# hellovuong/ORB_SLAM3_FAST

Measured on AMD Instinct MI355X. Metric: ORB extract+match frames/sec @1280×720 stereo (both-eye ORBextractor + ComputeStereoMatches), higher is better.
Workload: dtype u8; 1 GPU; C3: synthetic 1280x720 rectified stereo pairs, 1500 features, 8 levels, scale 1.2, FAST 20/7, ComputeStereoMatches (bf=0.12*532.03, b=0.12); handles=4, distinct_streams_per_gpu=32, frames_in_ring=3, stereo_matches_pair0=987, parallelism=independent stereo pairs sharded across GPUs, no data-path collective

## Files before the change

include/orbx.h:

```cpp
#ifndef ORBX_H_
#define ORBX_H_

#include <stddef.h>
#include <stdint.h>

#ifdef __cplusplus
extern "C" {
#endif

#define ORBX_MAX_LEVELS 12

#define ORBX_OK 0
#define ORBX_E_EMPTY (-1)
#define ORBX_E_BADARG (-2)
#define ORBX_E_CAPACITY (-3)
#define ORBX_E_HIP (-4)
#define ORBX_E_NODEVICE (-5)
#define ORBX_E_UNSUPPORTED (-6)
#define ORBX_E_TIMEOUT (-7)

typedef struct orbx_keypoint {
  float x, y, size, angle, response;
  int32_t octave, class_id;
} orbx_keypoint;
// ... 878 lines not shown
#define ORBX_GEOM_OPLUS 11
#define ORBX_GEOM_SIM3_EXP 12
#define ORBX_GEOM_SIM3_OPLUS 13
#define ORBX_GEOM_SO_INVERSE 14
#define ORBX_GEOM_RODRIGUES2ROT 15
#define ORBX_GEOM_ROT2RODRIGUES 16
#define ORBX_GEOM_OPS 17
#define ORBX_GEOM_MAX_ITEMS 65536
int orbx_debug_geometry(int device, int op, int n, const void* in, void* out);

void orbx_debug_set_detect_list_cap(int cap);
void orbx_debug_set_octree_global(int on);
void orbx_debug_set_octree_class(int nt);
int orbx_debug_octree_plan(const orbx_params* p, int width, int height, int32_t* nt_per_level, int32_t* lds_bytes_per_level);
void orbx_debug_set_stereo_direct(int max_pairs);
int orbx_debug_stereo_sort(orbx_extractor* left, int pair, int32_t* row_start, uint32_t* records, uint32_t* descriptors, int cap);
int orbx_debug_upload_results(orbx_extractor* ex, int image, const orbx_keypoint* kps, const uint8_t* desc, int n, int mono_index);
void orbx_debug_set_clahe_cell_kernel(int on);
void orbx_debug_set_remap_lds(int on);
int orbx_debug_remap_footprints(const float* map_x, const float* map_y, ptrdiff_t map_stride, int out_w, int out_h, int src_w,
                                int src_h, int n_maps, int32_t* table, int cap, int32_t* tiles_x, int32_t* tiles_y);
int orbx_debug_front_tables(const orbx_params* p, int width, int height, uint32_t* cells, int cells_cap, uint32_t* tiles,
                            int tiles_cap, int32_t info[4]);
int orbx_debug_preproc_plan(const orbx_preproc* pp, int32_t info[8]);
void orbx_debug_set_resize_tail(int first_level, int max_levels, int band_rows);
int orbx_debug_resize_plan(const orbx_extractor* ex, int32_t* first_level, int32_t* n_levels, int32_t* n_bands, int cap);
int orbx_debug_score_map(orbx_extractor* ex, int enable);
int orbx_debug_score_level(orbx_extractor* ex, int image, int level, uint8_t* dst, ptrdiff_t dst_stride);
int orbx_debug_sincos(int device, const float* angles, int n, int fused, float* sin_out, float* cos_out);
int orbx_debug_fast_atan2(int device, const float* y, const float* x, int n, float* out);
int orbx_debug_describe_plan(const orbx_params* p, int width, int height, int n_images, int32_t* out);
#define ORBX_SCRATCH_STATS 0
#define ORBX_SCRATCH_FILL 1
#define ORBX_SCRATCH_TRIM 2
int orbx_debug_scratch_pool(int device, int op, int byte, uint64_t* out);
int orbx_debug_fill_work_buffers(orbx_extractor* ex, int byte);

#ifdef __cplusplus
}
#endif
#endif
```

orb_slam3_fast_amd/__init__.py:

```python
import ctypes as C
import os

import numpy as np

_HERE = os.path.dirname(os.path.abspath(__file__))
LIB_PATH = os.path.join(_HERE, os.environ.get("ORBX_LIB_NAME", "liborbx.so"))

KP_DTYPE = np.dtype([("x", "<f4"), ("y", "<f4"), ("size", "<f4"), ("angle", "<f4"), ("response", "<f4"),
                     ("octave", "<i4"), ("class_id", "<i4")])
assert KP_DTYPE.itemsize == 28

OK, E_EMPTY, E_BADARG, E_CAPACITY, E_HIP, E_NODEVICE, E_UNSUPPORTED, E_TIMEOUT = 0, -1, -2, -3, -4, -5, -6, -7
TH_HIGH, TH_LOW, HISTO_LENGTH = 100, 50, 30
NUM_STAGES = 8
MP_DTYPE = np.dtype([("proj_x", "<f4"), ("proj_y", "<f4"), ("proj_xr", "<f4"), ("view_cos", "<f4"), ("track_depth", "<f4"),
                     ("predicted_level", "<i4"), ("in_view", "u1"), ("bad", "u1"), ("has_observations", "u1"),
                     ("pad_", "u1"), ("desc", "u1", (32,))])
assert MP_DTYPE.itemsize == 60
PP_DTYPE = np.dtype([("u", "<f4"), ("v", "<f4"), ("ur", "<f4"), ("radius", "<f4"), ("angle", "<f4"), ("min_level", "<i4"),
                     ("max_level", "<i4"), ("valid", "u1"), ("has_observations", "u1"), ("pad_", "u1", (2,)),
                     ("desc", "u1", (32,))])
assert PP_DTYPE.itemsize == 64
FP_DTYPE = np.dtype([("u", "<f4"), ("v", "<f4"), ("ur", "<f4"), ("radius", "<f4"), ("predicted_level", "<i4"), ("valid", "u1"),
                     ("pad_", "u1", (3,)), ("desc", "u1", (32,))])
# ... 186 lines not shown
                                                                       vp, vp]
        L.orbx_debug_inertial_linalg.argtypes = [i, i, i, vp, vp]
        L.orbx_debug_set_detect_list_cap.argtypes = [i]
        L.orbx_debug_set_detect_list_cap.restype = None
        L.orbx_debug_set_octree_global.argtypes = [i]
        L.orbx_debug_set_octree_global.restype = None
        if hasattr(L, "orbx_debug_set_octree_class"):
            L.orbx_debug_set_octree_class.argtypes = [i]
            L.orbx_debug_set_octree_class.restype = None
            L.orbx_debug_octree_plan.argtypes = [vp, i, i, vp, vp]
        L.orbx_debug_set_stereo_direct.argtypes = [i]
        L.orbx_debug_set_stereo_direct.restype = None
        if hasattr(L, "orbx_debug_stereo_sort"):
            L.orbx_debug_stereo_sort.argtypes = [vp, i, vp, vp, vp, i]
        L.orbx_debug_set_clahe_cell_kernel.argtypes = [i]
        L.orbx_debug_set_clahe_cell_kernel.restype = None
        L.orbx_debug_upload_results.argtypes = [vp, i, vp, vp, i, i]
        L.orbx_debug_set_remap_lds.argtypes = [i]
        L.orbx_debug_set_remap_lds.restype = None
        L.orbx_debug_remap_footprints.argtypes = [vp, vp, C.c_ssize_t, i, i, i, i, i, vp, i, C.POINTER(i), C.POINTER(i)]
        L.orbx_debug_preproc_plan.argtypes = [vp, vp]
        if hasattr(L, "orbx_debug_front_tables"):
            L.orbx_debug_front_tables.argtypes = [vp, i, i, vp, i, vp, i, vp]
        L.orbx_debug_set_resize_tail.argtypes = [i, i, i]
        L.orbx_debug_set_resize_tail.restype = None
        L.orbx_debug_resize_plan.argtypes = [vp, vp, vp, vp, i]
        L.orbx_debug_sincos.argtypes = [i, vp, i, i, vp, vp]
        if hasattr(L, "orbx_debug_fast_atan2"):
            L.orbx_debug_fast_atan2.argtypes = [i, vp, vp, i, vp]
            L.orbx_debug_describe_plan.argtypes = [vp, i, i, i, vp]
        L.orbx_debug_score_map.argtypes = [vp, i]
        L.orbx_set_opencv_compat.argtypes = [vp, i]
        L.orbx_debug_score_level.argtypes = [vp, i, i, vp, C.c_ssize_t]
        L.orbx_debug_scratch_pool.argtypes = [i, i, i, vp]
        L.orbx_debug_fill_work_buffers.argtypes = [vp, i]
        _lib = L
    return _lib


def _check(rc):
    if rc < 0:
        raise OrbxError(rc, lib().orbx_last_error().decode())
    return rc


def _p(a):
# ... 324 lines not shown
        _check(lib().orbx_debug_score_level(self._h, image, level, _p(out), w.value))
        return out

    def debug_resize_plan(self):
        a, b, c = (np.zeros(16, np.int32) for _ in range(3))
        n = _check(lib().orbx_debug_resize_plan(self._h, _p(a), _p(b), _p(c), 16))
        return [(int(a[i]), int(b[i]), int(c[i])) for i in range(n)]

    def debug_candidates(self, level, image=0):
        cap = 1 << 20
        out = np.zeros((cap, 3), np.int32)
        n = _check(lib().orbx_debug_candidates(self._h, image, level, _p(out), cap))
        return out[:n].copy()

    def debug_octree(self, width, height, candidates):
        counts, flat = _octree_candidates(candidates, self.nlevels)
        n = len(candidates)
        cap = int(self._nfeat.max()) + 64
        nsel = np.zeros(n * self.nlevels, np.int32)
        sel = np.zeros((n, self.nlevels, cap, 3), np.int32)
        _check(lib().orbx_debug_octree(self._h, int(width), int(height), n, _p(counts), _p(flat), _p(nsel), _p(sel), cap))
        return [[sel[i, l, :nsel[i * self.nlevels + l]].copy() for l in range(self.nlevels)] for i in range(n)]

    def debug_fill_work_buffers(self, byte):
        _check(lib().orbx_debug_fill_work_buffers(self._h, int(byte)))


SCRATCH_STATS, SCRATCH_FILL, SCRATCH_TRIM = 0, 1, 2


def scratch_pool_stats(device=0):
    out = np.zeros(4, np.uint64)
    _check(lib().orbx_debug_scratch_pool(int(device), SCRATCH_STATS, 0, _p(out)))
    return tuple(int(v) for v in out)


def scratch_pool_fill(byte, device=0):
    out = np.zeros(4, np.uint64)
    _check(lib().orbx_debug_scratch_pool(int(device), SCRATCH_FILL, int(byte), _p(out)))
    return int(out[0])


def scratch_pool_trim(device=0):
    _check(lib().orbx_debug_scratch_pool(int(device), SCRATCH_TRIM, 0, None))


# ... 1301 lines not shown
        raise ValueError("map_x and map_y must be float images of the same size")
    nm, dh, dw = mx.shape
    tx, ty = (dw + 127) // 128, (dh + 7) // 8
    tab = np.zeros((nm, tx, ty, 8), np.int32)
    gx, gy = C.c_int(), C.c_int()
    rc = lib().orbx_debug_remap_footprints(_p(mx), _p(my), dw, dw, dh, src_w, src_h, nm, _p(tab), tab.size, C.byref(gx), C.byref(gy))
    _check(rc)
    if (gx.value, gy.value) != (tx, ty):
        raise OrbxError("unexpected tile grid %d x %d" % (gx.value, gy.value))
    return tab if rc == 1 else None


def front_tables(nfeatures, scaleFactor, nlevels, iniThFAST, minThFAST, width, height):
    prm = _Params(int(nfeatures), float(scaleFactor), int(nlevels), int(iniThFAST), int(minThFAST))
    info = np.zeros(4, np.int32)
    _check(lib().orbx_debug_front_tables(C.byref(prm), width, height, None, 0, None, 0, _p(info)))
    cells = np.zeros((int(info[0]), 16), np.uint32)
    tiles = np.zeros(int(info[1]), np.uint32)
    _check(lib().orbx_debug_front_tables(C.byref(prm), width, height, _p(cells), cells.size, _p(tiles) if tiles.size else None,
                                         tiles.size, _p(info)))
    return cells, tiles, int(info[2]), int(info[3])


def octree_plan(nfeatures, scaleFactor, nlevels, iniThFAST, minThFAST, width, height):
    prm = _Params(int(nfeatures), float(scaleFactor), int(nlevels), int(iniThFAST), int(minThFAST))
    nt, lds = np.zeros(int(nlevels), np.int32), np.zeros(int(nlevels), np.int32)
    _check(lib().orbx_debug_octree_plan(C.byref(prm), width, height, _p(nt), _p(lds)))
    return nt, lds


def _octree_candidates(candidates, nlevels):
    counts, parts = [], [np.zeros((0, 3), np.int32)]
    for per_level in candidates:
        if len(per_level) != nlevels:
            raise ValueError("one candidate array per level")
        for c in per_level:
            c = np.asarray(c, np.int32).reshape(-1, 3)
            counts.append(len(c))
            parts.append(c)
    return np.array(counts, np.int32), np.ascontiguousarray(np.concatenate(parts))


def octree_check(nfeatures, scaleFactor, nlevels, iniThFAST, minThFAST, width, height, candidates):
    prm = _Params(int(nfeatures), float(scaleFactor), int(nlevels), int(iniThFAST), int(minThFAST))
    counts, flat = _octree_candidates(candidates, int(nlevels))
    _check(lib().orbx_debug_octree_check(C.byref(prm), int(width), int(height), len(candidates), _p(counts), _p(flat)))
# ... 521 lines not shown
```

orb_slam3_fast_amd/csrc/orbx_api.hip:

```cpp
#include "orbx_host.h"
#include "orbx_rgbd.h"

namespace orbx_host {
thread_local std::string g_err;
}

namespace {
struct StageTimer {
  orbx_extractor* ex;
  hipStream_t s;
  int stage;
  size_t i0 = 0;
  bool on;
  StageTimer(orbx_extractor* ex_, hipStream_t s_, int stage_)
      : ex(ex_), s(s_), stage(stage_), on(ex_->profiling && (ex_->profStage < 0 || ex_->profStage == stage_)) {
    if (!on) {
      if (s == ex->stream) ex->lastEvValid = false;
      return;
    }
    if (s == ex->stream && ex->lastEvValid) {
      i0 = ex->lastEv;
    } else {
      hipEvent_t e = ex->next_event();
      i0 = ex->evCursor - 1;
// ... 167 lines not shown
        const int ce = std::min((int)xtab[D.xcoef + x1].x + 1, S.w - 1);
        const int ndw = ((ce - cb) >> 2) + 1;
        const bool whole = l > 1 || cb + 4 * ndw <= S.w;
        const bool fast = whole && ndw > 64 && ndw <= 85 && nrows <= 24 && rb + 28 <= S.h;
        uint32_t* t = &tab[(size_t)tileOff + 8 * (size_t)(tby * nbx + tbx)];
        t[0] = (uint32_t)(D.xcoef + x0);
        t[1] = (uint32_t)x0 | ((uint32_t)(y1 - y0 + 1) << 16);
        t[2] = (uint32_t)rb | ((uint32_t)nrows << 16);
        t[3] = (uint32_t)cb | ((uint32_t)ndw << 16);
        t[4] = (fast ? kTileFast : 0u) | (whole ? kTileWhole : 0u);
        t[5] = (uint32_t)((long long)y0 * D.pitch);
        t[6] = (uint32_t)tby;
      }
      for (int w = 0; w < 4; w++)
        for (int k = 0; k < 4; k++) {
          const int dy = std::min(y0 + w + 4 * k, D.h - 1);
          const uint32_t sy = yrow[D.ycoef + dy];
          uint32_t* r = &tab[(size_t)rowOff + 16 * (size_t)(4 * tby + w) + 4 * k];
          r[0] = (uint32_t)(uint16_t)yab[2 * (D.ycoef + dy)] | ((uint32_t)(uint16_t)yab[2 * (D.ycoef + dy) + 1] << 16);
          r[1] = (uint32_t)(((int)(sy & 0xFFFFu) - rb) * 512);
          r[2] = (uint32_t)(((int)(sy >> 16) - rb) * 512);
        }
    }
  }
}

void build_cell_records(const Geom& g, std::vector<CellRec>& recs) {
  recs.assign((size_t)g.totalCells, CellRec{});
  const int TPd = g.tileP >> 2;
  for (int l = 0; l < g.nlevels; l++) {
    const LevelDev& L = g.lv[l];
    const int maxBX = L.w - kBorder, maxBY = L.h - kBorder;
    for (int ci = 0; ci < L.nRows; ci++)
      for (int cj = 0; cj < L.nCols; cj++) {
        const int cell = ci * L.nCols + cj;
        CellRec& r = recs[(size_t)L.cellStart + cell];
        const int iniY = kBorder + ci * L.hCell, iniX = kBorder + cj * L.wCell;
        const int maxY = std::min(iniY + L.hCell + 6, maxBY), maxX = std::min(iniX + L.wCell + 6, maxBX);
        const int rw = maxX - iniX, rh = maxY - iniY;
        const int dw = rw - 6, dh = rh - 6;
        r.flags = ((uint32_t)l << 8) | ((uint32_t)L.w << 16) | (l == 0 ? kCellL0 : 0u);
        if (iniY >= maxBY - 3 || iniX >= maxBX - 6 || dw <= 0 || dh <= 0) {
          r.flags |= kCellReject;
          continue;
        }
        if (iniX + g.tileP <= L.w) r.flags |= kCellWide;
// ... 209 lines not shown
  if (g.pyrImg > m.pyrImg || g.candImg > m.candImg || g.selImg > m.selImg || g.cellImg > m.cellImg ||
      g.totalCells > m.totalCells)
    return fail(ORBX_E_CAPACITY, "image within max_width x max_height but its pyramid / cell-grid rounding needs more "
                                 "buffer than the handle's maximum size: create the handle with this size");
  g.outCap = m.outCap;
  g.selImg = m.selImg;
  g.pyrImg = m.pyrImg;
  g.candImg = m.candImg;
  g.cellImg = m.cellImg;
  std::vector<uint4> xtab;
  std::vector<int> yofs;
  std::vector<short> yab;
  build_coefs(g, xtab, yofs, yab);
  HIPC(hipStreamSynchronize(ex->stream));
  HIPC(hipMemcpy(ex->d_xtab.p, xtab.data(), xtab.size() * sizeof(uint4), hipMemcpyHostToDevice));
  HIPC(hipMemcpy(ex->d_yofs.p, yofs.data(), yofs.size() * sizeof(int), hipMemcpyHostToDevice));
  {
    std::vector<uint32_t> yrow, rec;
    build_yrow(g, yofs, yrow);
    HIPC(hipMemcpy(ex->d_yrow.p, yrow.data(), yrow.size() * sizeof(uint32_t), hipMemcpyHostToDevice));
    build_resize_records(g, xtab, yrow, yab, rec);
    if (ex->d_rsRec.n < rec.size()) HIPC(ex->d_rsRec.alloc(rec.size()));
    if (!rec.empty()) HIPC(hipMemcpy(ex->d_rsRec.p, rec.data(), rec.size() * sizeof(uint32_t), hipMemcpyHostToDevice));
  }
  HIPC(hipMemcpy(ex->d_yab.p, yab.data(), yab.size() * sizeof(short), hipMemcpyHostToDevice));
  {
    std::vector<CellRec> recs;
    build_cell_records(g, recs);
    HIPC(hipMemcpy(ex->d_cellRec.p, recs.data(), recs.size() * sizeof(CellRec), hipMemcpyHostToDevice));
  }
  build_octree_plan(g, ex->octPlan);
  HIPC(prepare_kernels(g));
  std::vector<TailPlan> plans;
  std::vector<TailBand> bands;
  build_tail_plans(g, yofs, plans, bands);
  if (!plans.empty()) {
    if (ex->d_tailBands.n < bands.size()) HIPC(ex->d_tailBands.alloc(bands.size()));
    HIPC(hipMemcpy(ex->d_tailBands.p, bands.data(), bands.size() * sizeof(TailBand), hipMemcpyHostToDevice));
    unsigned lds = 0;
    for (const TailPlan& tp : plans) lds = std::max(lds, tp.ldsBytes);
    HIPC(prepare_resize_tail(lds));
  }
  ex->tails = plans;
  {
    std::vector<TailPlan> lp;
    std::vector<TailBand> lb;
// ... 77 lines not shown
      HIPC(hipMemcpyAsync(ex->d_lap.p, ex->h_lap, nb, hipMemcpyHostToDevice, s));
    }
  }
  return ORBX_OK;
}

static int enqueue_pyramid(orbx_extractor* ex, hipStream_t s, int img0, int n) {
  const Geom& g = ex->g;
  if (ex->useLat) {
    for (const TailPlan& tp : ex->latTails) {
      StageTimer t(ex, s, ORBX_STAGE_RESIZE);
      HIPC(launch_resize_tail(g, ex->pyr, tp, ex->d_latBands.p + tp.bandOff, img0, n, ex->d_xtab.p, ex->d_yofs.p, ex->d_yab.p, s));
    }
    return ORBX_OK;
  }
  size_t seg = 0;
  for (int l = 1; l < g.nlevels;) {
    StageTimer t(ex, s, ORBX_STAGE_RESIZE);
    if (seg < ex->tails.size() && ex->tails[seg].lA == l) {
      const TailPlan& tp = ex->tails[seg++];
      HIPC(launch_resize_tail(g, ex->pyr, tp, ex->d_tailBands.p + tp.bandOff, 0, n, ex->d_xtab.p, ex->d_yofs.p, ex->d_yab.p, s));
      l += tp.nT;
    } else {
      HIPC(launch_resize(g, ex->pyr, n, l, ex->d_xtab.p, ex->d_yrow.p, ex->d_yab.p, ex->d_rsRec.p, s));
      l++;
    }
  }
  return ORBX_OK;
}

int enqueue_extract(orbx_extractor* ex, const uint8_t* d_images, int n, int w, int h, ptrdiff_t row_pitch,
                    ptrdiff_t image_pitch, const int32_t* lap) {
  bool lapTrivial = true;
  int rc = prepare_extract(ex, d_images, n, w, h, row_pitch, image_pitch, lap, lapTrivial);
  if (rc != ORBX_OK) return rc;
  hipStream_t s = ex->stream;
  static const bool useGraph = env_int("ORBX_GRAPH", 0) != 0;
  if (useGraph && n == 1 && d_images == ex->d_stage.p && !ex->profiling && !ex->graphOff) {
    if (ex->graphW != w || ex->graphH != h) {
      drop_graphs(ex);
      ex->graphW = w;
      ex->graphH = h;
    }
    hipGraphExec_t& exec = ex->graphExec[lapTrivial ? 1 : 0];
    if (!exec) {
      hipGraph_t graph = nullptr;
      bool ok = hipStreamBeginCapture(s, hipStreamCaptureModeThreadLocal) == hipSuccess;
// ... 131 lines not shown
  ok(ex->d_cellCount.alloc(B * m.totalCells));
  ok(ex->d_cellPrefix.alloc(B * m.totalCells));
  ok(ex->d_knode.alloc(B * m.candImg));
  ok(ex->d_candCount.alloc(B * m.nlevels));
  ok(ex->d_sel.alloc(B * m.selImg));
  ok(ex->d_selCount.alloc(B * m.nlevels + ORBX_MAX_LEVELS));
  ok(ex->d_slot.alloc(B * m.selImg));
  ok(ex->d_kps.alloc(B * m.outCap));
  ok(ex->d_desc.alloc(B * m.outCap * 32));
  ok(ex->d_nOut.alloc(B));
  ok(ex->d_mono.alloc(B));
  ok(ex->d_lap.alloc(B * 2));
  ok(hipHostMalloc(reinterpret_cast<void**>(&ex->h_lap), (size_t)B * 2 * sizeof(int), hipHostMallocDefault));
  ok(ex->d_xtab.alloc(nx + 64));
  ok(ex->d_cellRec.alloc(m.totalCells));
  {
    int tiles = 0, trows = 0;
    for (int l = 1; l < m.nlevels; l++) {
      tiles += ((m.lv[l].w + 255) / 256 + 1) * ((m.lv[l].h + 15) / 16 + 1);
      trows += (m.lv[l].h + 15) / 16 + 1;
    }
    ok(ex->d_rsRec.alloc((size_t)8 * tiles + 64 * trows + 64));
  }
  ok(ex->d_yofs.alloc(ny + 64));
  ok(ex->d_yrow.alloc(ny + 64));
  ok(ex->d_packCtr.alloc(4));
  if (e == hipSuccess) e = hipMemset(ex->d_packCtr.p, 0, 4 * sizeof(int));
  ok(ex->d_yab.alloc(2 * ny + 64));
  ok(hipHostMalloc(reinterpret_cast<void**>(&ex->hostResults), host_results_bytes(m.outCap), hipHostMallocDefault));
  if (e != hipSuccess) {
    std::string msg = std::string("allocation failed: ") + hipGetErrorString(e);
    orbx_extractor_destroy(ex);
    return fail(ORBX_E_HIP, msg);
  }
  std::memset(ex->hostResults, 0, 64);
  *out = ex;
  return ORBX_OK;
}

void orbx_extractor_destroy(orbx_extractor* ex) {
  if (!ex) return;
  (void)hipSetDevice(ex->device);
  if (ex->stream) (void)hipStreamSynchronize(ex->stream);
  for (auto& e : ex->graphExec) {
    if (e) (void)hipGraphExecDestroy(e);
    e = nullptr;
// ... 735 lines not shown
  build_tables(ex.get());
  Geom g;
  std::string why;
  const int rc = build_geom(ex.get(), width, height, g, why);
  if (rc != ORBX_OK) return fail(rc, why);
  std::vector<uint4> xtab;
  std::vector<int> yofs;
  std::vector<short> yab;
  std::vector<uint32_t> yrow, rec;
  std::vector<CellRec> cr;
  build_coefs(g, xtab, yofs, yab);
  build_yrow(g, yofs, yrow);
  build_resize_records(g, xtab, yrow, yab, rec);
  build_cell_records(g, cr);
  info[0] = (int32_t)cr.size(); info[1] = (int32_t)rec.size(); info[2] = g.tileP; info[3] = g.tileH;
  if (cells) {
    if (cr.size() * 16 > (size_t)cells_cap) return fail(ORBX_E_CAPACITY, "cell records larger than cells_cap");
    std::memcpy(cells, cr.data(), cr.size() * sizeof(CellRec));
  }
  if (tiles) {
    if (rec.size() > (size_t)tiles_cap) return fail(ORBX_E_CAPACITY, "tile records larger than tiles_cap");
    std::memcpy(tiles, rec.data(), rec.size() * sizeof(uint32_t));
  }
  return ORBX_OK;
}

int orbx_debug_octree_plan(const orbx_params* p, int width, int height, int32_t* nt_per_level, int32_t* lds_bytes_per_level) {
  if (!p || !nt_per_level || !lds_bytes_per_level || width < 1 || height < 1 || p->nlevels < 1 || p->nlevels > ORBX_MAX_LEVELS ||
      p->nfeatures < 1 || !(p->scale_factor > 1.0f))
    return fail(ORBX_E_BADARG, "bad argument");
  std::unique_ptr<orbx_extractor> ex(new orbx_extractor());
  ex->prm = *p;
  build_tables(ex.get());
  Geom g;
  std::string why;
  const int rc = build_geom(ex.get(), width, height, g, why);
  if (rc != ORBX_OK) return fail(rc, why);
  OctPlan op;
  build_octree_plan(g, op);
  for (int l = 0; l < g.nlevels; l++) {
    nt_per_level[l] = op.nt[l];
    lds_bytes_per_level[l] = op.lds[l];
  }
  return ORBX_OK;
}

// ... 461 lines not shown
```

orb_slam3_fast_amd/csrc/orbx_host.h:

```cpp
#ifndef ORBX_HOST_H
#define ORBX_HOST_H
#if defined(__x86_64__) || defined(__i386__)
#include <immintrin.h>
static inline void cpu_pause() { _mm_pause(); }
#else
static inline void cpu_pause() {}
#endif
#include <memory>
#include <new>
#include <chrono>
#include <climits>
#include <cmath>
#include <cstdio>
#include <cstdlib>
#include <cstring>
#include <string>
#include <mutex>
#include <type_traits>
#include <vector>

#include "orbx_internal.h"

namespace orbx {
inline const char* env_str(const char* name) { return getenv(name); }
inline bool env_set(const char* name) { return env_str(name) != nullptr; }
inline int env_int(const char* name, int dflt) {
  const char* e = env_str(name);
  return e ? atoi(e) : dflt;
}
}

using namespace orbx;

namespace orbx_host {


extern thread_local std::string g_err;
void build_coefs(const Geom& g, std::vector<uint4>& xtab, std::vector<int>& yofs, std::vector<short>& yab);
void build_cell_records(const Geom& g, std::vector<CellRec>& recs);
void build_yrow(const Geom& g, const std::vector<int>& yofs, std::vector<uint32_t>& yrow);
void build_resize_records(const Geom& g, const std::vector<uint4>& xtab, const std::vector<uint32_t>& yrow, const std::vector<short>& yab,
                          std::vector<uint32_t>& tab);
inline int fail(int code, const std::string& msg) {
  g_err = msg;
  return code;
}
inline double trace_slow_ms() {
  static const double v = env_set("ORBX_TRACE_SLOW") ? atof(env_str("ORBX_TRACE_SLOW")) : 0.0;
  return v;
}
#define HIPC(expr)                                                                                     \
  do {                                                                                                 \
    const double lim_ = trace_slow_ms();                                                               \
    const auto t0_ = lim_ > 0 ? std::chrono::steady_clock::now() : std::chrono::steady_clock::time_point(); \
    hipError_t e_ = (expr);                                                                            \
    if (lim_ > 0) {                                                                                    \
      const double ms_ = std::chrono::duration<double, std::milli>(std::chrono::steady_clock::now() - t0_).count(); \
      if (ms_ > lim_) std::fprintf(stderr, "ORBX_TRACE_SLOW %.2f ms: %s (%s:%d)\n", ms_, #expr, __FILE__, __LINE__); \
    }                                                                                                  \
    if (e_ != hipSuccess)                                                                              \
      return fail(ORBX_E_HIP, std::string(#expr) + ": " + hipGetErrorString(e_));                      \
  } while (0)

inline int cv_round(float v) { return (int)lrintf(v); }
inline int cv_round(double v) { return (int)lrint(v); }
// ... 309 lines not shown

struct orbx_extractor {
  orbx_params prm{};
  int device = 0;
  hipStream_t stream = nullptr;
  hipEvent_t done = nullptr;
  int maxW = 0, maxH = 0, maxB = 0;
  std::vector<float> scale, inv, sig2, invsig2;
  std::vector<int> nfeat;
  int umax[16];
  Geom g{};
  Geom gmax{};
  int curW = 0, curH = 0;
  Pyr pyr{};
  int lastN = 0;
  DevBuf<uint8_t> d_pyr, d_blur, d_stage, d_desc;
  DevBuf<uint8_t> d_dbgScore;
  DevBuf<uint32_t> d_cand, d_cellCand, d_sel;
  DevBuf<uint16_t> d_knode;
  DevBuf<int> d_rowStart, d_cellCount, d_cellPrefix, d_candCount, d_selCount, d_slot, d_nOut, d_mono, d_lap, d_yofs, d_sad;
  DevBuf<short> d_yab;
  DevBuf<uint4> d_xtab;
  DevBuf<uint32_t> d_rsRec;
  DevBuf<orbx::CellRec> d_cellRec;
  orbx::OctPlan octPlan{};
  DevBuf<int> d_packCtr;
  uint32_t packSeq = 0;
  bool packCtrDirty = false;
  DevBuf<uint32_t> d_yrow;
  DevBuf<uint4> d_srec, d_sdesc;
  std::vector<orbx::TailPlan> tails;
  DevBuf<orbx::TailBand> d_tailBands;
  std::vector<orbx::TailPlan> latTails;
  DevBuf<orbx::TailBand> d_latBands;
  DevBuf<orbx_keypoint> d_kps;
  DevBuf<float> d_uR, d_depth;
  int stagePitch = 0;
  int stereoPairs = 0;
  int lastStereoPairs = 0;
  int uRPairs = 0;
  DevBuf<float> d_mapPos, d_mapNormal, d_mapMinD, d_mapMaxD;
  DevBuf<uint8_t> d_mapDesc, d_mapFlags, d_mapSkip;
  DevBuf<orbx_frame_pose> d_poses;
  DevBuf<orbx_map_point_view> d_views;
  DevBuf<float> d_lfPos, d_lfAngle;
  DevBuf<int> d_lfOct, d_lfN;
// ... 56 lines not shown
  WORK(d_pyr)                                                          \
  WORK(d_blur)                                        \
  WORK(d_stage)                                                            \
  WORK(d_desc)                                                                             \
  WORK(d_dbgScore)                                 \
  WORK(d_cand)                                                                           \
  WORK(d_cellCand)                                                              \
  WORK(d_sel)                                                                            \
  WORK(d_knode)                                                               \
  WORK(d_rowStart)                                     \
  WORK(d_cellCount)                                                                      \
  WORK(d_cellPrefix)                                                                   \
  WORK(d_candCount)                                                           \
  WORK(d_selCount)        \
  WORK(d_slot)                                                          \
  WORK(d_nOut)                                                               \
  WORK(d_mono)                                                              \
  UPLOAD(d_lap)                                             \
  TABLE(d_yofs)                                                                               \
  WORK(d_sad)                                              \
  TABLE(d_yab)                                                                           \
  TABLE(d_xtab)                                                                          \
  TABLE(d_rsRec)                                                                             \
  TABLE(d_cellRec)                                                                       \
  STATE(d_packCtr)                                    \
  TABLE(d_yrow)                                                                  \
  WORK(d_srec)                                             \
  WORK(d_sdesc)                                                                           \
  TABLE(d_tailBands)                                                              \
  TABLE(d_latBands)                                                                      \
  WORK(d_kps)                                                                                \
  WORK(d_uR)                                                            \
  WORK(d_depth)                                                                                             \
  UPLOAD(d_mapPos) UPLOAD(d_mapNormal) UPLOAD(d_mapMinD) UPLOAD(d_mapMaxD)                          \
  UPLOAD(d_mapDesc) UPLOAD(d_mapFlags)                                                                                   \
  UPLOAD(d_mapSkip)                                                  \
  UPLOAD(d_poses)                                                                                         \
  WORK(d_views)                                             \
  UPLOAD(d_lfPos) UPLOAD(d_lfAngle) UPLOAD(d_lfOct) UPLOAD(d_lfN) UPLOAD(d_lfDesc) UPLOAD(d_lfFlags)    \
  UPLOAD(d_posesQ)                                                          \
  WORK(d_pviews)                                                                                    \
  UPLOAD(d_scaleF)                                                                   \
  UPLOAD(d_posesK)                                                           \
  WORK(d_fviewsL) WORK(d_fviewsR)                                                                \
  WORK(d_bowWord) WORK(d_bowNode) WORK(d_bowStart) WORK(d_bowCounts)      \
  WORK(d_bowWeight) WORK(d_bowValues) WORK(d_bowWords) WORK(d_bowNodes) WORK(d_bowFeats)                                 \
// ... 34 lines not shown
```

orb_slam3_fast_amd/csrc/orbx_internal.h:

```cpp
#pragma once
#include <hip/hip_runtime.h>
#include <stdint.h>
#include <vector>

#include "../../include/orbx.h"

namespace orbx {

constexpr int kEdge = 19;
constexpr int kHalfPatch = 15;
constexpr int kBorder = 16;
constexpr int kMaxIni = 8;

struct LevelDev {
  int w, h, pitch;
  int nCols, nRows, wCell, hCell;
  int cellStart;
  int quota;
  int candCap;
  int cellCap;
  int selOff, selCap;
  int xcoef, ycoef;
  long long off;
  long long candOff;
// ... 71 lines not shown
  int first, last, ownEnd, pad_;
};
struct TailPlan {
  int lA, nT, nBands, bandOff;
  int tileBytes[2];
  int pitch[ORBX_MAX_LEVELS + 1];
  int rtOff[ORBX_MAX_LEVELS];
  int rtTotal;
  unsigned ldsBytes;
};
hipError_t launch_resize_tail(const Geom& g, const Pyr& p, const TailPlan& tp, const TailBand* bands, int img0, int nimg,
                              const uint4* xtab, const int* yofs, const short* yab, hipStream_t s);
hipError_t prepare_resize_tail(unsigned ldsBytes);
hipError_t raise_dynamic_lds(const void* fn, size_t bytes);

size_t resize_plain_lds(int sw, int sh, int dw, int dh);
hipError_t prepare_resize_plain(int sw, int sh, int dw, int dh);
hipError_t launch_resize_plain(const uint8_t* src, int sw, int sh, long long sp, long long sip, uint8_t* dst, int dw, int dh,
                               long long dp, long long dip, const uint4* xtab, const uint32_t* yrow, const short* yab, int nimg,
                               hipStream_t s);
hipError_t launch_resize(const Geom& g, const Pyr& p, int nimg, int level, const uint4* xtab, const uint32_t* yofs ,
                         const short* yab, const uint32_t* records, hipStream_t s);
int resize_records_layout(const Geom& g, int level, int& tileOff, int& rowOff);
constexpr uint32_t kTileFast = 1u, kTileWhole = 2u;
hipError_t launch_detect(const Geom& g, const Pyr& p, const CellRec* cellRec, int nimg, uint32_t* cellCand, int* cellCount,
                         int level0, int level1, uint8_t* dbgScore, hipStream_t s);
hipError_t launch_octree(const Geom& g, int nimg, const uint32_t* cellCand, const int* cellCount, int* cellPrefix,
                         uint32_t* cand, int* candCount, uint16_t* knode, uint32_t* sel, int* selCount, int level0,
                         int level1, int nt, hipStream_t s);
struct OctPlan {
  int nt[ORBX_MAX_LEVELS], lds[ORBX_MAX_LEVELS];
};
void build_octree_plan(const Geom& g, OctPlan& p);
hipError_t launch_octree_mixed(const Geom& g, const OctPlan& plan, int nimg, const uint32_t* cellCand, const int* cellCount,
                               uint32_t* cand, int* candCount, uint16_t* knode, uint32_t* sel, int* selCount, hipStream_t s);
hipError_t launch_blur(const Geom& g, const Pyr& p, int nimg, int level0, int level1, hipStream_t s);
hipError_t launch_slots(const Geom& g, int nimg, const uint32_t* sel, const int* selCount, const int* lap,
                        int* slot, int* nOut, int* mono, hipStream_t s);
hipError_t launch_describe(const Geom& g, const Pyr& p, int nimg, const uint32_t* sel, const int* selCount,
                           const int* slot, orbx_keypoint* kps, uint8_t* desc, int* nOut, int* mono, hipStream_t s);
size_t octree_lds_bytes(const Geom& g, int level0, int level1);
size_t resize_lds_bytes(const Geom& g);

struct StereoArgs {
  const orbx_keypoint *kL, *kR;
  const uint8_t *dL, *dR;
// ... 385 lines not shown
```

orb_slam3_fast_amd/csrc/orbx_resize.hip:

```cpp
#include "orbx_device.h"
#include "orbx_prof.h"

namespace orbx {

#define RS_DW 256
#define RS_DR 16
#define RS_HROWS 6
struct ResizeLv {
  struct { int w, h, pitch, xcoef, ycoef; } D;
  struct { int w, h; } S;
  int sp, l;
  int nbx;
  const uint8_t* src; long long srcImg;
  uint8_t* dst; long long dstImg;
  const uint32_t* tiles;
  const uint32_t* rows;
};
constexpr int kResizeXcdRun = 8;
__device__ __forceinline__ uint32_t vblend4(uint2 t0, uint2 t1, uint32_t bb, uint32_t kRound) {
  uint32_t p0, p1, p2, p3, q0, q1, q2, q3, w01, w23;
  asm("v_mad_u32_u16 %0, %1, %2, %3" : "=v"(p0) : "v"(t0.x), "s"(bb), "v"(kRound));
  asm("v_mad_u32_u16 %0, %1, %2, %3 op_sel:[1,0,0,0]" : "=v"(p1) : "v"(t0.x), "s"(bb), "v"(kRound));
  asm("v_mad_u32_u16 %0, %1, %2, %3" : "=v"(p2) : "v"(t0.y), "s"(bb), "v"(kRound));
  asm("v_mad_u32_u16 %0, %1, %2, %3 op_sel:[1,0,0,0]" : "=v"(p3) : "v"(t0.y), "s"(bb), "v"(kRound));
// ... 300 lines not shown
hipError_t prepare_resize_plain(int sw, int sh, int dw, int dh) {
  const size_t lds = std::max<size_t>(resize_plain_lds(sw, sh, dw, dh), 1024);
  hipError_t e = raise_dynamic_lds(reinterpret_cast<const void*>(k_resize<0, false>), lds);
  if (e == hipSuccess) e = raise_dynamic_lds(reinterpret_cast<const void*>(k_resize<kResizeNdw, false>), lds);
  return e;
}
hipError_t launch_resize_plain(const uint8_t* src, int sw, int sh, long long sp, long long sip, uint8_t* dst, int dw, int dh,
                               long long dp, long long dip, const uint4* xtab, const uint32_t* yrow, const short* yab, int nimg,
                               hipStream_t s) {
  const Geom g = resize_plain_geom(sw, sh, dw, dh, dp, dip);
  Pyr p{};
  p.l0 = src; p.l0Row = sp; p.l0Img = sip; p.pyr = dst;
  return launch_resize(g, p, nimg, 1, xtab, yrow, yab, nullptr, s);
}

hipError_t prepare_resize(const Geom& g) {
  if (g.nlevels <= 1) return hipSuccess;
  const size_t lds = std::max<size_t>(resize_lds_bytes(g), 1024);
  hipError_t e = raise_dynamic_lds(reinterpret_cast<const void*>(k_resize<0, true>), lds);
  if (e == hipSuccess) e = raise_dynamic_lds(reinterpret_cast<const void*>(k_resize<kResizeNdw, true>), lds);
  return e;
}

}
```

Measured before the change: 85960 stereo frames/s.

## Add streaming per-strip resize kernel with precomputed lane tables for batched pyramids

Adds a new pyramid resize kernel in which each lane owns a quad of output columns in a strip. The lane loads one unaligned 8-byte source window per row, selects pixels by byte-permute with precomputed selectors, and streams down a band of rows with double-buffered row loads, emitting vertical blends as output rows complete. Host-built lane tables (selectors, coefficients, offsets) are uploaded at setup. The kernel is used in place of the tiled LDS resize only when the batch exceeds the latency image threshold and the offset limits hold. It is meant to cut LDS staging and record indirection, at the risk of unaligned global loads and redundant row reads at band edges.

```diff
diff --git a/include/orbx.h b/include/orbx.h
--- a/include/orbx.h
+++ b/include/orbx.h
@@ -924,6 +924,10 @@
                                 int src_h, int n_maps, int32_t* table, int cap, int32_t* tiles_x, int32_t* tiles_y);
 int orbx_debug_front_tables(const orbx_params* p, int width, int height, uint32_t* cells, int cells_cap, uint32_t* tiles,
                             int tiles_cap, int32_t info[4]);
+int orbx_debug_resize_stream_tables(const orbx_params* p, int width, int height, int quads, uint32_t* lanes, int lanes_cap,
+                                    int32_t* level_off);
+int orbx_debug_resize_stream(orbx_extractor* ex, const uint8_t* d_images, int n_images, int w, int h, ptrdiff_t row_pitch,
+                             ptrdiff_t image_pitch, int kernel, int quads, int band);
 int orbx_debug_preproc_plan(const orbx_preproc* pp, int32_t info[8]);
 void orbx_debug_set_resize_tail(int first_level, int max_levels, int band_rows);
 int orbx_debug_resize_plan(const orbx_extractor* ex, int32_t* first_level, int32_t* n_levels, int32_t* n_bands, int cap);
diff --git a/orb_slam3_fast_amd/__init__.py b/orb_slam3_fast_amd/__init__.py
--- a/orb_slam3_fast_amd/__init__.py
+++ b/orb_slam3_fast_amd/__init__.py
@@ -232,6 +232,9 @@
         L.orbx_debug_preproc_plan.argtypes = [vp, vp]
         if hasattr(L, "orbx_debug_front_tables"):
             L.orbx_debug_front_tables.argtypes = [vp, i, i, vp, i, vp, i, vp]
+        if hasattr(L, "orbx_debug_resize_stream"):
+            L.orbx_debug_resize_stream_tables.argtypes = [vp, i, i, i, vp, i, vp]
+            L.orbx_debug_resize_stream.argtypes = [vp, vp, i, i, i, C.c_ssize_t, C.c_ssize_t, i, i, i]
         L.orbx_debug_set_resize_tail.argtypes = [i, i, i]
         L.orbx_debug_set_resize_tail.restype = None
         L.orbx_debug_resize_plan.argtypes = [vp, vp, vp, vp, i]
@@ -602,6 +605,10 @@
         _check(lib().orbx_debug_octree(self._h, int(width), int(height), n, _p(counts), _p(flat), _p(nsel), _p(sel), cap))
         return [[sel[i, l, :nsel[i * self.nlevels + l]].copy() for l in range(self.nlevels)] for i in range(n)]
 
+    def debug_resize_stream(self, d_images_ptr, n_images, w, h, row_pitch, image_pitch, kernel=1, quads=0, band=0):
+        _check(lib().orbx_debug_resize_stream(self._h, C.c_void_p(d_images_ptr), int(n_images), int(w), int(h), int(row_pitch),
+                                              int(image_pitch), int(kernel), int(quads), int(band)))
+
     def debug_fill_work_buffers(self, byte):
         _check(lib().orbx_debug_fill_work_buffers(self._h, int(byte)))
 
@@ -1949,6 +1956,17 @@
     return cells, tiles, int(info[2]), int(info[3])
 
 
+def resize_stream_tables(nfeatures, scaleFactor, nlevels, iniThFAST, minThFAST, width, height, quads=64):
+    prm = _Params(int(nfeatures), float(scaleFactor), int(nlevels), int(iniThFAST), int(minThFAST))
+    off = np.zeros(12, np.int32)
+    n = _check(lib().orbx_debug_resize_stream_tables(C.byref(prm), width, height, quads, None, 0, _p(off)))
+    tab = np.zeros(n, np.uint32)
+    _check(lib().orbx_debug_resize_stream_tables(C.byref(prm), width, height, quads, _p(tab) if n else None, n, _p(off)))
+    ends = sorted([int(o) for o in off if o >= 0] + [n])
+    return [tab[o:ends[ends.index(int(o)) + 1]].reshape(-1, 3, quads, 4) if l < nlevels and o >= 0 else None
+            for l, o in enumerate(off[:nlevels])]
+
+
 def octree_plan(nfeatures, scaleFactor, nlevels, iniThFAST, minThFAST, width, height):
     prm = _Params(int(nfeatures), float(scaleFactor), int(nlevels), int(iniThFAST), int(minThFAST))
     nt, lds = np.zeros(int(nlevels), np.int32), np.zeros(int(nlevels), np.int32)
diff --git a/orb_slam3_fast_amd/csrc/orbx_api.hip b/orb_slam3_fast_amd/csrc/orbx_api.hip
--- a/orb_slam3_fast_amd/csrc/orbx_api.hip
+++ b/orb_slam3_fast_amd/csrc/orbx_api.hip
@@ -213,6 +213,42 @@
           r[2] = (uint32_t)(((int)(sy >> 16) - rb) * 512);
         }
     }
+  }
+}
+
+void build_resize_stream(const Geom& g, const std::vector<uint4>& xtab, int quads, std::vector<uint4>& tab, int* laneOff) {
+  tab.clear();
+  for (int l = 0; l < ORBX_MAX_LEVELS; l++) laneOff[l] = -1;
+  for (int l = 1; l < g.nlevels; l++) {
+    const LevelDev &D = g.lv[l], &S = g.lv[l - 1];
+    const int nq = (D.w + 3) / 4, nStrips = (nq + quads - 1) / quads;
+    if (S.w < 8) continue;
+    std::vector<uint4> lv((size_t)nStrips * 3 * quads);
+    bool ok = true;
+    for (int qi = 0; qi < nStrips * quads && ok; qi++) {
+      const int qv = std::min(qi, nq - 1);
+      const uint4* e = &xtab[(size_t)D.xcoef + 4 * qv];
+      int lo = (int)e[0].x, hi = lo;
+      for (int j = 0; j < 4; j++) {
+        lo = std::min(lo, (int)e[j].x);
+        hi = std::max(hi, std::min((int)e[j].x + 1, S.w - 1));
+      }
+      const int off = std::min(lo, S.w - 8);
+      if (hi - off > 7) { ok = false; break; }
+      uint32_t sel[4], cf[4];
+      for (int j = 0; j < 4; j++) {
+        const uint32_t b0 = (uint32_t)((int)e[j].x - off), b1 = (uint32_t)(std::min((int)e[j].x + 1, S.w - 1) - off);
+        sel[j] = b0 | 0x0c000c00u | (b1 << 16);
+        cf[j] = e[j].w;
+      }
+      uint4* o = &lv[(size_t)(qi / quads) * 3 * quads + qi % quads];
+      o[0] = make_uint4(sel[0], sel[1], sel[2], sel[3]);
+      o[quads] = make_uint4(cf[0], cf[1], cf[2], cf[3]);
+      o[2 * quads] = make_uint4((uint32_t)off, qi < nq ? (uint32_t)(4 * qi) : 0xFFFFFFFFu, 0u, 0u);
+    }
+    if (!ok) continue;
+    laneOff[l] = (int)tab.size();
+    tab.insert(tab.end(), lv.begin(), lv.end());
   }
 }
 
@@ -468,6 +504,10 @@
     build_resize_records(g, xtab, yrow, yab, rec);
     if (ex->d_rsRec.n < rec.size()) HIPC(ex->d_rsRec.alloc(rec.size()));
     if (!rec.empty()) HIPC(hipMemcpy(ex->d_rsRec.p, rec.data(), rec.size() * sizeof(uint32_t), hipMemcpyHostToDevice));
+    std::vector<uint4> lanes;
+    build_resize_stream(g, xtab, kStreamQuads, lanes, ex->rsStreamOff);
+    if (ex->d_rsStream.n < lanes.size()) return fail(ORBX_E_CAPACITY, "lane tables larger than the handle's maximum size allows");
+    if (!lanes.empty()) HIPC(hipMemcpy(ex->d_rsStream.p, lanes.data(), lanes.size() * sizeof(uint4), hipMemcpyHostToDevice));
   }
   HIPC(hipMemcpy(ex->d_yab.p, yab.data(), yab.size() * sizeof(short), hipMemcpyHostToDevice));
   {
@@ -591,7 +631,11 @@
       HIPC(launch_resize_tail(g, ex->pyr, tp, ex->d_tailBands.p + tp.bandOff, 0, n, ex->d_xtab.p, ex->d_yofs.p, ex->d_yab.p, s));
       l += tp.nT;
     } else {
-      HIPC(launch_resize(g, ex->pyr, n, l, ex->d_xtab.p, ex->d_yrow.p, ex->d_yab.p, ex->d_rsRec.p, s));
+      if (n > g_lat_max_images && resize_stream_ok(g, ex->pyr, l, kStreamQuads, ex->rsStreamOff))
+        HIPC(launch_resize_stream(g, ex->pyr, n, l, ex->d_rsStream.p + ex->rsStreamOff[l], kStreamQuads, kStreamBand, ex->d_yrow.p,
+                                  ex->d_yab.p, s));
+      else
+        HIPC(launch_resize(g, ex->pyr, n, l, ex->d_xtab.p, ex->d_yrow.p, ex->d_yab.p, ex->d_rsRec.p, s));
       l++;
     }
   }
@@ -769,6 +813,11 @@
     }
     ok(ex->d_rsRec.alloc((size_t)8 * tiles + 64 * trows + 64));
   }
+  {
+    size_t lanes = 0;
+    for (int l = 1; l < m.nlevels; l++) lanes += (size_t)(((m.lv[l].w + 3) / 4 + kStreamQuads - 1) / kStreamQuads + 1) * 3 * kStreamQuads;
+    ok(ex->d_rsStream.alloc(lanes + 64));
+  }
   ok(ex->d_yofs.alloc(ny + 64));
   ok(ex->d_yrow.alloc(ny + 64));
   ok(ex->d_packCtr.alloc(4));
@@ -1550,6 +1599,76 @@
     if (rec.size() > (size_t)tiles_cap) return fail(ORBX_E_CAPACITY, "tile records larger than tiles_cap");
     std::memcpy(tiles, rec.data(), rec.size() * sizeof(uint32_t));
   }
+  return ORBX_OK;
+}
+
+int orbx_debug_resize_stream_tables(const orbx_params* p, int width, int height, int quads, uint32_t* lanes, int lanes_cap,
+                                    int32_t* level_off) {
+  if (!p || !level_off || width < 1 || height < 1 || lanes_cap < 0 || (lanes_cap && !lanes) || (quads != 32 && quads != 64) ||
+      p->nlevels < 1 || p->nlevels > ORBX_MAX_LEVELS || p->nfeatures < 1 || !(p->scale_factor > 1.0f))
+    return fail(ORBX_E_BADARG, "bad argument");
+  std::unique_ptr<orbx_extractor> ex(new orbx_extractor());
+  ex->prm = *p;
+  build_tables(ex.get());
+  Geom g;
+  std::string why;
+  const int rc = build_geom(ex.get(), width, height, g, why);
+  if (rc != ORBX_OK) return fail(rc, why);
+  std::vector<uint4> xtab, tab;
+  std::vector<int> yofs;
+  std::vector<short> yab;
+  int off[ORBX_MAX_LEVELS];
+  build_coefs(g, xtab, yofs, yab);
+  build_resize_stream(g, xtab, quads, tab, off);
+  for (int l = 0; l < ORBX_MAX_LEVELS; l++) level_off[l] = off[l] < 0 ? -1 : 4 * off[l];
+  if (lanes) {
+    if (tab.size() * 4 > (size_t)lanes_cap) return fail(ORBX_E_CAPACITY, "lane tables larger than lanes_cap");
+    if (!tab.empty()) std::memcpy(lanes, tab.data(), tab.size() * sizeof(uint4));
+  }
+  return (int)(tab.size() * 4);
+}
+
+int orbx_debug_resize_stream(orbx_extractor* ex, const uint8_t* d_images, int n_images, int w, int h, ptrdiff_t row_pitch,
+                             ptrdiff_t image_pitch, int kernel, int quads, int band) {
+  if (!ex) return fail(ORBX_E_BADARG, "null handle");
+  if (!d_images || n_images <= 0 || w <= 0 || h <= 0) return fail(ORBX_E_EMPTY, "empty image");
+  if (n_images > ex->maxB) return fail(ORBX_E_CAPACITY, "batch larger than max_batch");
+  if (row_pitch < w || (kernel != 0 && kernel != 1)) return fail(ORBX_E_BADARG, "bad argument");
+  if (kernel == 0 && (((uintptr_t)d_images & 3) || (row_pitch & 3) || (image_pitch & 3)))
+    return fail(ORBX_E_BADARG, "k_resize needs 4-byte aligned images and pitches");
+  if (quads == 0) quads = kStreamQuads;
+  if (band == 0) band = kStreamBand;
+  if ((quads != 32 && quads != 64) || band < 1 || band > 4096) return fail(ORBX_E_BADARG, "strips of 32 or 64 quads, bands of 1 .. 4096 rows");
+  int rc = set_device(ex->device);
+  if (rc != ORBX_OK) return rc;
+  bool lapTrivial = true;
+  rc = prepare_extract(ex, d_images, n_images, w, h, row_pitch, image_pitch, nullptr, lapTrivial);
+  if (rc != ORBX_OK) return rc;
+  const Geom& g = ex->g;
+  hipStream_t s = ex->stream;
+  DevBuf<uint4> d_lanes;
+  int off[ORBX_MAX_LEVELS];
+  if (kernel == 1) {
+    std::vector<uint4> xtab, tab;
+    std::vector<int> yofs;
+    std::vector<short> yab;
+    build_coefs(g, xtab, yofs, yab);
+    build_resize_stream(g, xtab, quads, tab, off);
+    for (int l = 1; l < g.nlevels; l++)
+      if (!resize_stream_ok(g, ex->pyr, l, quads, off)) return fail(ORBX_E_UNSUPPORTED, "level " + std::to_string(l) + " cannot stream");
+    if (!tab.empty()) {
+      HIPC(d_lanes.alloc(tab.size()));
+      HIPC(hipMemcpyAsync(d_lanes.p, tab.data(), tab.size() * sizeof(uint4), hipMemcpyHostToDevice, s));
+      HIPC(hipStreamSynchronize(s));
+    }
+  }
+  for (int l = 1; l < g.nlevels; l++) {
+    if (kernel == 1)
+      HIPC(launch_resize_stream(g, ex->pyr, n_images, l, d_lanes.p + off[l], quads, band, ex->d_yrow.p, ex->d_yab.p, s));
+    else
+      HIPC(launch_resize(g, ex->pyr, n_images, l, ex->d_xtab.p, ex->d_yrow.p, ex->d_yab.p, ex->d_rsRec.p, s));
+  }
+  HIPC(hipStreamSynchronize(s));
   return ORBX_OK;
 }
 
diff --git a/orb_slam3_fast_amd/csrc/orbx_host.h b/orb_slam3_fast_amd/csrc/orbx_host.h
--- a/orb_slam3_fast_amd/csrc/orbx_host.h
+++ b/orb_slam3_fast_amd/csrc/orbx_host.h
@@ -41,6 +41,7 @@
 void build_yrow(const Geom& g, const std::vector<int>& yofs, std::vector<uint32_t>& yrow);
 void build_resize_records(const Geom& g, const std::vector<uint4>& xtab, const std::vector<uint32_t>& yrow, const std::vector<short>& yab,
                           std::vector<uint32_t>& tab);
+void build_resize_stream(const Geom& g, const std::vector<uint4>& xtab, int quads, std::vector<uint4>& tab, int* laneOff);
 inline int fail(int code, const std::string& msg) {
   g_err = msg;
   return code;
@@ -396,6 +397,8 @@
   DevBuf<short> d_yab;
   DevBuf<uint4> d_xtab;
   DevBuf<uint32_t> d_rsRec;
+  DevBuf<uint4> d_rsStream;
+  int rsStreamOff[ORBX_MAX_LEVELS] = {};
   DevBuf<orbx::CellRec> d_cellRec;
   orbx::OctPlan octPlan{};
   DevBuf<int> d_packCtr;
@@ -498,6 +501,7 @@
   TABLE(d_yab)                                                                           \
   TABLE(d_xtab)                                                                          \
   TABLE(d_rsRec)                                                                             \
+  TABLE(d_rsStream)                                                                    \
   TABLE(d_cellRec)                                                                       \
   STATE(d_packCtr)                                    \
   TABLE(d_yrow)                                                                  \
diff --git a/orb_slam3_fast_amd/csrc/orbx_internal.h b/orb_slam3_fast_amd/csrc/orbx_internal.h
--- a/orb_slam3_fast_amd/csrc/orbx_internal.h
+++ b/orb_slam3_fast_amd/csrc/orbx_internal.h
@@ -117,6 +117,10 @@
 hipError_t launch_resize(const Geom& g, const Pyr& p, int nimg, int level, const uint4* xtab, const uint32_t* yofs ,
                          const short* yab, const uint32_t* records, hipStream_t s);
 int resize_records_layout(const Geom& g, int level, int& tileOff, int& rowOff);
+constexpr int kStreamQuads = 32, kStreamBand = 16;
+bool resize_stream_ok(const Geom& g, const Pyr& p, int level, int quads, const int* laneOff);
+hipError_t launch_resize_stream(const Geom& g, const Pyr& p, int nimg, int level, const uint4* lanes, int quads, int band,
+                                const uint32_t* yrow, const short* yab, hipStream_t s);
 constexpr uint32_t kTileFast = 1u, kTileWhole = 2u;
 hipError_t launch_detect(const Geom& g, const Pyr& p, const CellRec* cellRec, int nimg, uint32_t* cellCand, int* cellCount,
                          int level0, int level1, uint8_t* dbgScore, hipStream_t s);
diff --git a/orb_slam3_fast_amd/csrc/orbx_resize.hip b/orb_slam3_fast_amd/csrc/orbx_resize.hip
--- a/orb_slam3_fast_amd/csrc/orbx_resize.hip
+++ b/orb_slam3_fast_amd/csrc/orbx_resize.hip
@@ -346,4 +346,118 @@
   return e;
 }
 
-}
+struct __attribute__((packed, aligned(1))) ResizeU64Unaligned { uint32_t x, y; };
+struct StreamLv {
+  const uint8_t* src; long long srcImg; int sp;
+  uint8_t* dst; long long dstImg; int dpitch;
+  int dh, ycoef;
+  int nStrips, band, nimg;
+  const uint4* lanes;
+};
+constexpr int kStreamRows = 4;
+template <int QS>
+__global__ __launch_bounds__(64) void k_resize_stream(StreamLv a, const uint32_t* __restrict__ yrow, const uint32_t* __restrict__ yab) {
+  static_assert(QS == 64 || QS == 32, "a strip is a wave or a half-wave of quads");
+  constexpr int K = kStreamRows;
+  const int lane = threadIdx.x;
+  const int q = lane & (QS - 1), half = QS == 32 ? lane >> 5 : 0;
+  const int tIdx = xcd_run_remap<kResizeXcdRun>((int)blockIdx.x, (int)gridDim.x, (int)blockIdx.z);
+  const int bandI = __builtin_amdgcn_readfirstlane((int)(((float)tIdx + 0.5f) * __builtin_amdgcn_rcpf((float)a.nStrips)));
+  const int strip = tIdx - bandI * a.nStrips;
+  const int img0 = (int)blockIdx.z * (64 / QS);
+  const uint4* lt = a.lanes + (size_t)strip * (3 * QS) + q;
+  const uint4 sel = lt[0], coef = lt[QS], misc = lt[2 * QS];
+  if (misc.y == 0xFFFFFFFFu || img0 + half >= a.nimg) return;
+  const uint32_t soff = misc.x + (uint32_t)half * (uint32_t)a.srcImg;
+  const uint32_t doff = misc.y + (uint32_t)half * (uint32_t)a.dstImg;
+  const int y0 = bandI * a.band, y1 = min(y0 + a.band, a.dh) - 1;
+  const uint32_t* yr = yrow + a.ycoef;
+  const uint32_t* yb = yab + a.ycoef;
+  const int rb = (int)(yr[y0] & 0xFFFFu), re = (int)(yr[y1] >> 16);
+  const uint8_t* srcImg = a.src + (long long)img0 * a.srcImg;
+  uint8_t* dstRow = a.dst + (long long)img0 * a.dstImg + (long long)y0 * a.dpitch;
+  uint32_t kRound = 0x20000u;
+  asm volatile("" : "+v"(kRound));
+  int dy = y0;
+  uint32_t n0rr = yr[y0], n0bb = yb[y0];
+  uint32_t n1rr = yr[min(y0 + 1, y1)], n1bb = yb[min(y0 + 1, y1)];
+  uint2 cur = make_uint2(0u, 0u), prev = cur;
+  auto load = [&](uint2 (&v)[K], int r) {
+#pragma unroll
+    for (int k = 0; k < K; k++) {
+      const uint32_t o = soff + (uint32_t)(min(r + k, re) * a.sp);
+      const ResizeU64Unaligned t = *reinterpret_cast<const ResizeU64Unaligned*>(srcImg + o);
+      v[k] = make_uint2(t.x, t.y);
+    }
+  };
+  auto use = [&](const uint2 (&v)[K], int r) {
+#pragma unroll
+    for (int k = 0; k < K; k++) {
+      const int rk = r + k;
+      if (rk > re) break;
+      const uint32_t t0 = udot2_u16(__builtin_amdgcn_perm(v[k].y, v[k].x, sel.x), coef.x, 0u);
+      const uint32_t t1 = udot2_u16(__builtin_amdgcn_perm(v[k].y, v[k].x, sel.y), coef.y, 0u);
+      const uint32_t t2 = udot2_u16(__builtin_amdgcn_perm(v[k].y, v[k].x, sel.z), coef.z, 0u);
+      const uint32_t t3 = udot2_u16(__builtin_amdgcn_perm(v[k].y, v[k].x, sel.w), coef.w, 0u);
+      prev = cur;
+      cur.x = t0 >> 4;
+      cur.y = t2 >> 4;
+      asm("v_lshrrev_b32_sdwa %0, 4, %1 dst_sel:WORD_1 dst_unused:UNUSED_PRESERVE src0_sel:DWORD src1_sel:DWORD" : "+v"(cur.x) : "v"(t1));
+      asm("v_lshrrev_b32_sdwa %0, 4, %1 dst_sel:WORD_1 dst_unused:UNUSED_PRESERVE src0_sel:DWORD src1_sel:DWORD" : "+v"(cur.y) : "v"(t3));
+      while (dy <= y1 && (int)(n0rr >> 16) == rk) {
+        const bool same = (n0rr & 0xFFFFu) == (n0rr >> 16);
+        const uint32_t outw = vblend4(same ? cur : prev, cur, n0bb, kRound);
+        asm volatile("global_store_dword %0, %1, %2" : : "v"(doff), "v"(outw), "s"(dstRow) : "memory");
+        dstRow += a.dpitch;
+        dy++;
+        n0rr = n1rr, n0bb = n1bb;
+        const int nx = min(dy + 1, y1);
+        n1rr = yr[nx], n1bb = yb[nx];
+      }
+    }
+  };
+  uint2 A[K], B[K];
+  load(A, rb);
+  for (int r = rb;; r += 2 * K) {
+    if (r + K > re) { use(A, r); break; }
+    load(B, r + K);
+    use(A, r);
+    if (r + 2 * K > re) { use(B, r + K); break; }
+    load(A, r + 2 * K);
+    use(B, r + K);
+  }
+}
+
+bool resize_stream_ok(const Geom& g, const Pyr& p, int level, int quads, const int* laneOff) {
+  if (level < 1 || level >= g.nlevels || laneOff[level] < 0) return false;
+  const long long sp = level == 1 ? p.l0Row : g.lv[level - 1].pitch, si = level == 1 ? p.l0Img : g.pyrImg;
+  const long long lim = 1ll << 31;
+  if (sp < 0 || sp * g.lv[level - 1].h >= lim) return false;
+  if (quads == 32 && (si < 0 || si + sp * g.lv[level - 1].h >= lim || g.pyrImg + (long long)g.lv[level].pitch * g.lv[level].h >= lim)) return false;
+  return true;
+}
+
+hipError_t launch_resize_stream(const Geom& g, const Pyr& p, int nimg, int level, const uint4* lanes, int quads, int band,
+                                const uint32_t* yrow, const short* yab, hipStream_t s) {
+  const LevelDev &D = g.lv[level], &S = g.lv[level - 1];
+  StreamLv a;
+  if (level == 1) {
+    a.src = p.l0; a.srcImg = p.l0Img; a.sp = (int)p.l0Row;
+  } else {
+    a.src = p.pyr + S.off; a.srcImg = g.pyrImg; a.sp = S.pitch;
+  }
+  a.dst = p.pyr + D.off; a.dstImg = g.pyrImg; a.dpitch = D.pitch;
+  a.dh = D.h; a.ycoef = D.ycoef;
+  a.nStrips = ((D.w + 3) / 4 + quads - 1) / quads;
+  a.band = band;
+  a.nimg = nimg;
+  a.lanes = lanes;
+  const int nBands = (D.h + band - 1) / band;
+  const dim3 grid(a.nStrips * nBands, 1, quads == 32 ? (nimg + 1) / 2 : nimg);
+  const uint32_t* yabw = reinterpret_cast<const uint32_t*>(yab);
+  if (quads == 32) hipLaunchKernelGGL(k_resize_stream<32>, grid, dim3(64), 0, s, a, yrow, yabw);
+  else hipLaunchKernelGGL(k_resize_stream<64>, grid, dim3(64), 0, s, a, yrow, yabw);
+  return hipGetLastError();
+}
+
+}
```

Measured after the change: 88680 stereo frames/s (median of 6 runs). 1.03x the previous value.
